# Hanbo-Cheng/DAWN-pytorch

Hardware: NVIDIA H100
Metric: denoising-steps/sec (200-frame 256^2 clip) (higher is better)
Workload: dtype f32

## Files before the change

dawn_pytorch_b200/_lib.py:

```python
import ctypes
import os

_HERE = os.path.dirname(os.path.abspath(__file__))
LIB_PATH = os.path.join(_HERE, "libdawn_unet.so")


class DawnUnetCfg(ctypes.Structure):
    _fields_ = [("dim", ctypes.c_int), ("n_levels", ctypes.c_int), ("dim_mults", ctypes.c_int * 8),
                ("channels", ctypes.c_int), ("cond_aud", ctypes.c_int), ("cond_pose", ctypes.c_int),
                ("cond_eye", ctypes.c_int), ("out_grid_dim", ctypes.c_int), ("out_conf_dim", ctypes.c_int),
                ("attn_heads", ctypes.c_int), ("attn_dim_head", ctypes.c_int), ("resnet_groups", ctypes.c_int),
                ("init_kernel_size", ctypes.c_int), ("win_width", ctypes.c_int)]


class DawnLfgCfg(ctypes.Structure):
    _fields_ = [("num_channels", ctypes.c_int), ("block_expansion", ctypes.c_int), ("max_features", ctypes.c_int),
                ("num_down_blocks", ctypes.c_int), ("num_bottleneck_blocks", ctypes.c_int), ("skips", ctypes.c_int)]


PATH_MMA_SYNC, PATH_TC_GEMM, PATH_TC_GEMM_PRESPLIT, PATH_TC_CONV3, PATH_TC_CONV3_TMA = range(5)
EPI_PLAIN, EPI_QKV_TEMPORAL, EPI_QKV_SLA, EPI_QKV_MID, EPI_CA_GATE, EPI_GN_APPLY = range(6)


class DawnContractionCase(ctypes.Structure):
    _i, _p = ctypes.c_int, ctypes.c_void_p
    _fields_ = [("path", _i), ("epi", _i),
                ("F", _i), ("IH", _i), ("IW", _i), ("Cin", _i), ("lda", _i),
                ("ntaps", _i), ("dy", _i * 52), ("dx", _i * 52), ("in_stride", _i),
                ("OHs", _i), ("OWs", _i), ("OH", _i), ("OW", _i), ("out_stride", _i), ("oy0", _i), ("ox0", _i),
                ("up2", _i),
                ("perm_pb", _i), ("perm_F", _i), ("perm_in", _i), ("perm_out", _i), ("perm_f_lo", _i), ("perm_f_hi", _i),
                ("P", _i),
                ("N", _i), ("ldb", _i), ("ldo", _i), ("ldr", _i), ("drain", _i), ("ln_inline", _i),
                ("rows_per_batch", _i), ("b_batch_stride", ctypes.c_longlong), ("cpg", _i),
                ("q_post_scale", ctypes.c_float),
                ("A", _p), ("B", _p), ("bias", _p), ("Res", _p), ("Out", _p),
                ("stats", _p), ("rowstats", _p), ("wsum", _p), ("rot", _p),
                ("kq", _p), ("nkq", _p), ("gates", _p),
                ("Y", _p), ("ldy", _i), ("gn_stats", _p), ("gn_w", _p), ("gn_b", _p), ("film", _p), ("gn_count", ctypes.c_double)]


FUSED_TEMPORAL, FUSED_ATTN_TC, FUSED_ATTN_SIMT, FUSED_SLA_CTX, FUSED_SLA_OUT, FUSED_SLA_CTX_UNFUSED, FUSED_CA_WT, \
    FUSED_CA_RSTD, FUSED_GN_HCOND, FUSED_TEMPORAL_MMA_SYNC = range(10)


class DawnFusedCase(ctypes.Structure):
    _i, _p = ctypes.c_int, ctypes.c_void_p
    _fields_ = [("kernel", _i), ("F", _i), ("P", _i), ("C", _i), ("band", _i), ("q_lo", _i), ("q_hi", _i),
                ("nseq", _i), ("L", _i), ("pb", _i), ("seq_base_stride", ctypes.c_longlong), ("elem_stride", ctypes.c_longlong),
                ("ldx", _i), ("ldr", _i), ("ldo", _i), ("ld", _i), ("ldb", _i), ("ldy", _i), ("ldbT", _i),
                ("x", _p), ("res", _p), ("out", _p), ("gamma", _p), ("w_qkv", _p), ("w_out", _p), ("rot", _p), ("bias", _p),
                ("qkv", _p), ("Bf", _p), ("out_bias", _p), ("kq", _p), ("nkq", _p), ("G", _p), ("gates", _p), ("Wt", _p),
                ("T", _p), ("Y", _p), ("out16h", _p), ("out16l", _p),
                ("gn_stats", _p), ("gn_count", ctypes.c_double), ("cpg", _i), ("gn_w", _p), ("gn_b", _p), ("film", _p)]
# ... 182 lines not shown
```

dawn_pytorch_b200/csrc/contraction.cu:

```cuda
#include <algorithm>
#include <cstring>

#include "common.cuh"
#include "contraction.cuh"
#include "kernels.cuh"
#include "tc_gemm.cuh"

namespace dawn {

void HostParams::set(const std::string& name, const float* data, const int64_t* shape, int ndim) {
  HostParam p;
  p.shape.assign(shape, shape + ndim);
  int64_t numel = 1;
  for (int64_t s : p.shape) numel *= s;
  p.data.assign(data, data + numel);
  map[name] = std::move(p);
}

int HostParams::need(const std::string& name, const std::vector<int64_t>& shape, const HostParam** out) const {
  auto it = map.find(name);
  if (it == map.end()) { set_last_error(prefix + "missing parameter: " + name); return -1; }
  const HostParam& p = it->second;
  if (p.shape != shape) {
    std::string s = prefix + "parameter " + name + " has shape (";
// ... 217 lines not shown

  GemmParams p;
  memset(&p, 0, sizeof(p));
  p.A = c.A; p.lda = c.lda; p.Cin = c.Cin;
  p.up2 = c.up2;
  p.IH = c.IH; p.IW = c.IW; p.OHs = c.OHs; p.OWs = c.OWs; p.in_stride = c.in_stride;
  p.ntaps = c.ntaps;
  for (int t = 0; t < c.ntaps; ++t) { p.dy[t] = (signed char)c.dy[t]; p.dx[t] = (signed char)c.dx[t]; }
  p.M = c.F * c.OHs * c.OWs; p.N = c.N; p.K = c.ntaps * c.Cin;
  p.rows_per_batch = c.rows_per_batch > 0 ? c.rows_per_batch : p.M;
  p.perm_pb = c.perm_pb; p.perm_F = c.perm_F; p.perm_in = c.perm_in; p.perm_out = c.perm_out;
  p.perm_f_lo = c.perm_f_lo; p.perm_f_hi = c.perm_f_hi;
  p.B = c.B; p.ldb = c.ldb; p.b_batch_stride = c.b_batch_stride;
  p.Out = c.Out; p.ldo = c.ldo; p.OH = c.OH; p.OW = c.OW; p.out_stride = c.out_stride; p.oy0 = c.oy0; p.ox0 = c.ox0;
  p.bias = c.bias; p.Res = c.Res; p.ldr = c.ldr;
  p.stats = c.stats; p.cpg = c.cpg; p.clips = 1;
  p.rowstats = c.rowstats; p.ln_inline = c.ln_inline; p.wsum = c.wsum; p.rot = c.rot; p.P = c.P;
  p.q_post_scale = c.q_post_scale;
  p.kq = c.kq; p.nkq = c.nkq; p.gates = c.gates;
  p.Y = c.Y; p.ldy = c.ldy; p.gn_stats = c.gn_stats; p.gn_w = c.gn_w; p.gn_b = c.gn_b; p.film = c.film; p.gn_count = c.gn_count;
  p.drain = c.drain;

  const bool ln = c.epi >= EPI_QKV_TEMPORAL && c.epi <= EPI_CA_GATE;
  if (p.ln_inline && (c.path != DAWN_PATH_TC_GEMM || p.ntaps != 1)) return refuse("inline LayerNorm statistics need the gather-producer wgmma GEMM and one tap");
  if (ln && !p.ln_inline && !p.rowstats) return refuse("LayerNorm epilogue without row statistics");
  if (ln && !p.wsum) return refuse("LayerNorm epilogue without wsum");
  if (c.epi == EPI_PLAIN && p.stats && (p.cpg <= 0 || p.N / p.cpg > 8)) return refuse("GroupNorm statistics need 8 groups");

  Owned own;
  if (c.path != DAWN_PATH_MMA_SYNC) {
    std::vector<float> hB((size_t)p.K * p.ldb);
    DAWN_CUDA_OK(cudaMemcpy(hB.data(), p.B, hB.size() * sizeof(float), cudaMemcpyDeviceToHost));
    PackedWeight w;
    DAWN_TRY(upload_weight(own.v, hB, p.K, p.N, p.ldb, {}, &w));
    set_weights(p, w);
    p.bias = c.bias;
  }
  const bool split = c.path == DAWN_PATH_TC_GEMM_PRESPLIT || c.path == DAWN_PATH_TC_CONV3_TMA;
  const size_t scratch_bytes = split ? (size_t)split_rows(p) * p.Cin * 4 : 0;
  if (!path_ok(p, c.epi, c.path, scratch_bytes)) return refuse("the path does not accept this geometry");
  float* scratch = nullptr;
  if (split) DAWN_TRY(dev_alloc(own.v, scratch_bytes / sizeof(float), &scratch));
// ... 13 lines not shown
```

dawn_pytorch_b200/csrc/tc_common.cuh:

```cuda
#pragma once
#include <type_traits>
#include "common.cuh"

namespace dawn {
namespace tc {

__device__ __forceinline__ uint32_t smem_u32(const void* p) { return (uint32_t)__cvta_generic_to_shared(p); }

__device__ __forceinline__ uint8_t* smem_align1024(uint8_t* base) { return base + ((1024u - (smem_u32(base) & 1023u)) & 1023u); }

template <uint32_t R>
__device__ __forceinline__ void setmaxnreg_dec() { asm volatile("setmaxnreg.dec.sync.aligned.u32 %0;" ::"n"(R)); }
template <uint32_t R>
__device__ __forceinline__ void setmaxnreg_inc() { asm volatile("setmaxnreg.inc.sync.aligned.u32 %0;" ::"n"(R)); }

template <int I, int N, class F>
__device__ __forceinline__ void static_for(F&& f) {
  if constexpr (I < N) {
    f(std::integral_constant<int, I>{});
    static_for<I + 1, N>(f);
  }
}

__device__ __forceinline__ void mbar_init(uint64_t* bar, uint32_t count) {
// ... 59 lines not shown
      "setp.ne.b32 p, %50, 0;\n\t"
      "wgmma.mma_async.sync.aligned.m64n96k16.f32.f16.f16 "
      "{%0, %1, %2, %3, %4, %5, %6, %7, %8, %9, %10, %11, %12, %13, %14, %15, "
      "%16, %17, %18, %19, %20, %21, %22, %23, %24, %25, %26, %27, %28, %29, %30, %31, "
      "%32, %33, %34, %35, %36, %37, %38, %39, %40, %41, %42, %43, %44, %45, %46, %47}, %48, %49, p, 1, 1, 0, 0;\n\t"
      "}"
      : "+f"(d[0]), "+f"(d[1]), "+f"(d[2]), "+f"(d[3]), "+f"(d[4]), "+f"(d[5]), "+f"(d[6]), "+f"(d[7]), "+f"(d[8]), "+f"(d[9]),
        "+f"(d[10]), "+f"(d[11]), "+f"(d[12]), "+f"(d[13]), "+f"(d[14]), "+f"(d[15]), "+f"(d[16]), "+f"(d[17]), "+f"(d[18]),
        "+f"(d[19]), "+f"(d[20]), "+f"(d[21]), "+f"(d[22]), "+f"(d[23]), "+f"(d[24]), "+f"(d[25]), "+f"(d[26]), "+f"(d[27]),
        "+f"(d[28]), "+f"(d[29]), "+f"(d[30]), "+f"(d[31]), "+f"(d[32]), "+f"(d[33]), "+f"(d[34]), "+f"(d[35]), "+f"(d[36]),
        "+f"(d[37]), "+f"(d[38]), "+f"(d[39]), "+f"(d[40]), "+f"(d[41]), "+f"(d[42]), "+f"(d[43]), "+f"(d[44]), "+f"(d[45]),
        "+f"(d[46]), "+f"(d[47])
      : "l"(adesc), "l"(bdesc), "r"(scale_d)
      : "memory");
}
__device__ __forceinline__ void wgmma_m64n64k16_rs(float (&d)[32], const uint32_t (&a)[4], uint64_t bdesc, uint32_t scale_d) {
  asm volatile(
      "{\n\t"
      ".reg .pred p;\n\t"
      "setp.ne.b32 p, %37, 0;\n\t"
      "wgmma.mma_async.sync.aligned.m64n64k16.f32.f16.f16 "
      "{%0, %1, %2, %3, %4, %5, %6, %7, %8, %9, %10, %11, %12, %13, %14, %15, "
      "%16, %17, %18, %19, %20, %21, %22, %23, %24, %25, %26, %27, %28, %29, %30, %31}, {%32, %33, %34, %35}, %36, p, 1, 1, 0;\n\t"
      "}"
      : "+f"(d[0]), "+f"(d[1]), "+f"(d[2]), "+f"(d[3]), "+f"(d[4]), "+f"(d[5]), "+f"(d[6]), "+f"(d[7]), "+f"(d[8]), "+f"(d[9]),
        "+f"(d[10]), "+f"(d[11]), "+f"(d[12]), "+f"(d[13]), "+f"(d[14]), "+f"(d[15]), "+f"(d[16]), "+f"(d[17]), "+f"(d[18]),
        "+f"(d[19]), "+f"(d[20]), "+f"(d[21]), "+f"(d[22]), "+f"(d[23]), "+f"(d[24]), "+f"(d[25]), "+f"(d[26]), "+f"(d[27]),
        "+f"(d[28]), "+f"(d[29]), "+f"(d[30]), "+f"(d[31])
      : "r"(a[0]), "r"(a[1]), "r"(a[2]), "r"(a[3]), "l"(bdesc), "r"(scale_d)
      : "memory");
}

__device__ __forceinline__ uint64_t make_desc(uint32_t saddr, uint32_t sbo = 1024) {
  return (uint64_t)((saddr >> 4) & 0x3FFF) | (1ull << 16) | ((uint64_t)((sbo >> 4) & 0x3FFF) << 32) | (1ull << 62);
}

constexpr int kStageLd = 68;
__device__ __forceinline__ void stage_fragment(float* stage, int r0, const float (&d)[32], bool first, int wtid) {
  const int w = wtid >> 5, l = wtid & 31;
  float* p0 = stage + (size_t)(r0 + w * 16 + (l >> 2)) * kStageLd + 2 * (l & 3);
  float* p1 = p0 + 8 * kStageLd;
#pragma unroll
  for (int j = 0; j < 8; ++j) {
    float2* a = reinterpret_cast<float2*>(p0 + 8 * j);
    float2* b = reinterpret_cast<float2*>(p1 + 8 * j);
    if (first) {
      *a = make_float2(d[4 * j], d[4 * j + 1]);
      *b = make_float2(d[4 * j + 2], d[4 * j + 3]);
    } else {
      const float2 x = *a, y = *b;
      *a = make_float2(x.x + d[4 * j], x.y + d[4 * j + 1]);
      *b = make_float2(y.x + d[4 * j + 2], y.y + d[4 * j + 3]);
    }
  }
}

__device__ __forceinline__ uint32_t swz(int r, int c) { return (uint32_t)((r >> 3) * 1024 + (r & 7) * 128 + ((c ^ (r & 7)) << 4)); }

__device__ __forceinline__ void store_rows_coalesced(float* wbuf, const float (&acc)[64], float* out, size_t opix, int ldo,
                                                     int n0, bool rv, int lane) {
  float* dst[4];
#pragma unroll
  for (int k = 0; k < 4; ++k) {
    const int r = (lane >> 2) + 8 * k;
    const uint32_t lo = __shfl_sync(0xffffffffu, (uint32_t)opix, r);
    const uint32_t hi = __shfl_sync(0xffffffffu, (uint32_t)((unsigned long long)opix >> 32), r);
    const int ok = __shfl_sync(0xffffffffu, rv ? 1 : 0, r);
// ... 23 lines not shown
```

dawn_pytorch_b200/csrc/tc_conv3.cu:

```cuda
#include <cuda.h>
#include <cuda_fp16.h>
#include <cstdlib>
#include <cstring>
#include <string>
#include <map>
#include <tuple>
#include "common.cuh"
#include "f16x3.cuh"
#include "gemm.cuh"
#include "tc_common.cuh"
#include "tc_gemm.cuh"

namespace dawn {
namespace {

using namespace tc;

constexpr int TH = 16, TW = 8;
constexpr int HH = TH + 2, HW = TW + 2;
constexpr int NPROD = 256;
constexpr int PAIR_HH = 8 + 2;
constexpr int PAIR_ROW_B = 104;

template <int BN, bool PAIR = false>
struct CCfg {
  static_assert(!PAIR || BN == 64, "the pair-mode halos fit next to 64-column weight stages only");
  static constexpr int NWG = BN / 64;
  static constexpr bool SPLIT_EPI = (BN == 64);
  static constexpr int B_PANEL = BN * 128;
  static constexpr int FRAME_ROWS = PAIR ? PAIR_HH * HW : HH * HW;
  static constexpr int HALO_ROWS = PAIR ? PAIR_ROW_B + FRAME_ROWS : FRAME_ROWS;
  static constexpr int A_HALO = (HALO_ROWS * 128 + 1023) / 1024 * 1024;
  static constexpr int A_STAGES = 2;
  static constexpr int B_STAGES = PAIR ? 3 : (BN == 64) ? 4 : 2;
  static constexpr int A_BYTES = A_STAGES * 2 * A_HALO;
  static constexpr int B_BYTES = B_STAGES * 2 * B_PANEL;
  static constexpr int ACC_STAGE = 2 * 128 * kStageLd * 4;
  static constexpr int SMEM_DYN = A_BYTES + B_BYTES + ACC_STAGE + 1024;
  static_assert(SMEM_DYN + 1024 <= 232448, "shared memory");
  static constexpr int EPI_WARP = NPROD / 32 + 4 * NWG;
  static constexpr int LOAD_WARP = EPI_WARP + (SPLIT_EPI ? 4 : 0);
  static constexpr int NTHREADS = 32 * LOAD_WARP + 128;
  static constexpr uint32_t REG_LAUNCH = (65536 / NTHREADS) & ~7u;
  static constexpr uint32_t REG_LOAD = 24, REG_MMA = SPLIT_EPI ? 136 : 128, REG_EPI = 128;
  static_assert(REG_LOAD < REG_LAUNCH && REG_MMA > REG_LAUNCH && REG_EPI > REG_LAUNCH, "register budgets");
  static_assert(2 * REG_LAUNCH + REG_LOAD + NWG * REG_MMA + (SPLIT_EPI ? REG_EPI : 0) <= NTHREADS / 128 * REG_LAUNCH, "CTA register pool");
};

template <int BN, bool TMA, bool PAIR>
__device__ __forceinline__ void tc_conv3_body(const GemmParams& p, const float* __restrict__ Bimg, int tiles_y, int tiles_x, int tiles_n,
                                              int img_bn, const CUtensorMap& tm_hi, const CUtensorMap& tm_lo) {
  using C = CCfg<BN, PAIR>;
  constexpr int B_PANEL = C::B_PANEL, A_STAGES = C::A_STAGES, B_STAGES = C::B_STAGES, NWG = C::NWG;
  constexpr int A_HALO = C::A_HALO, FRAME_ROWS = C::FRAME_ROWS;
  constexpr bool SPLIT = C::SPLIT_EPI;
  extern __shared__ uint8_t smem_raw[];
  __shared__ uint64_t a_full[A_STAGES], a_free[A_STAGES], b_full[B_STAGES], b_free[B_STAGES];
  __shared__ uint64_t st_full[2], st_free[2];
  __shared__ float s_stat[NWG][16];
  __shared__ __align__(16) float s_bias[NWG][64];

  const int tid = threadIdx.x, lane = tid & 31;
  const int warp = __shfl_sync(0xffffffffu, tid >> 5, 0);
  uint8_t* smem = smem_align1024(smem_raw);
  uint8_t* smemA = smem;
  uint8_t* smemB = smem + C::A_BYTES;
  float* stage_base = reinterpret_cast<float*>(smemB + C::B_BYTES);

  if (tid == 0) {
    for (int s = 0; s < A_STAGES; ++s) { mbar_init(&a_full[s], TMA ? 1 : NPROD); mbar_init(&a_free[s], 4 * NWG); }
    for (int s = 0; s < B_STAGES; ++s) { mbar_init(&b_full[s], 1); mbar_init(&b_free[s], 4 * NWG); }
    for (int s = 0; s < 2; ++s) { mbar_init(&st_full[s], 128); mbar_init(&st_free[s], 128); }
    asm volatile("fence.mbarrier_init.release.cluster;" ::: "memory");
  }
  __syncthreads();
// ... 134 lines not shown
            if (PAIR) {
              bulk_copy_g2s(smemB + s * 2 * B_PANEL, panel, B_PANEL, &b_full[s]);
              bulk_copy_g2s(smemB + s * 2 * B_PANEL + B_PANEL, panel + ipanel, B_PANEL, &b_full[s]);
            } else {
              bulk_copy_g2s(smemB + s * 2 * B_PANEL, panel, 2 * B_PANEL, &b_full[s]);
            }
          }
      }
    }
    return;
  }

  const int wg = SPLIT ? 0 : (warp - 8) >> 2;
  const int ew = (warp - 8) & 3;
  const int etid = ew * 32 + lane;
  const int bar_id = 2 + wg;
  constexpr uint32_t SBO_HALO = HW * 128;
  constexpr uint32_t H2 = PAIR ? PAIR_ROW_B * 128 : 8 * HW * 128;
  const int dt = (p.drain == 1 || p.drain == 3) ? p.drain : 9;

  auto mma_tile = [&](auto DTc, float* stage, uint32_t& ait, uint32_t& bit, auto&& claim) {
    constexpr int DT = decltype(DTc)::value;
    float d0[32], d1[32];
    bool first_drain = true;
    for (int cc = 0; cc < NCH; ++cc, ++ait) {
      const int sa = ait % A_STAGES;
      mbar_wait(&a_full[sa], (ait / A_STAGES) & 1);
      fence_proxy_async();
      const uint32_t a_hi = smem_u32(smemA + sa * 2 * A_HALO), a_lo = a_hi + A_HALO;
      static_for<0, 9>([&](auto TAPc) {
        constexpr int tap = decltype(TAPc)::value;
        constexpr bool group_first = tap % DT == 0, group_last = tap % DT == DT - 1;
        constexpr uint32_t woff = (uint32_t)(((tap / 3) * HW + tap % 3) * 128);
        const int sb = bit % B_STAGES;
        const int sprev = (bit + B_STAGES - 1) % B_STAGES;
        mbar_wait(&b_full[sb], (bit / B_STAGES) & 1);
        const uint64_t ahi = make_desc(a_hi + woff, SBO_HALO), alo = make_desc(a_lo + woff, SBO_HALO);
        const uint64_t ahi2 = make_desc(a_hi + woff + H2, SBO_HALO), alo2 = make_desc(a_lo + woff + H2, SBO_HALO);
        const uint32_t sbaddr = smem_u32(smemB + sb * 2 * B_PANEL) + wg * 64 * 128;
        const uint64_t bhi = make_desc(sbaddr), blo = make_desc(sbaddr + B_PANEL);
        wgmma_fence();
#pragma unroll
        for (int j = 0; j < 4; ++j) {
          const uint64_t o = (uint64_t)(j * 2);
          const uint32_t acc = (group_first && j == 0) ? 0u : 1u;
          wgmma_m64n64k16(d0, alo + o, bhi + o, acc);
          wgmma_m64n64k16(d1, alo2 + o, bhi + o, acc);
          wgmma_m64n64k16(d0, ahi + o, blo + o, 1u);
          wgmma_m64n64k16(d1, ahi2 + o, blo + o, 1u);
          wgmma_m64n64k16(d0, ahi + o, bhi + o, 1u);
          wgmma_m64n64k16(d1, ahi2 + o, bhi + o, 1u);
        }
        wgmma_commit();
        if constexpr (group_last) {
          wgmma_wait<0>();
          wgmma_fence_acc(d0); wgmma_fence_acc(d1);
          if (lane == 0) { if (!group_first) mbar_arrive(&b_free[sprev]); mbar_arrive(&b_free[sb]); }
          if (first_drain) claim();
          stage_fragment(stage, 0, d0, first_drain, etid);
          stage_fragment(stage, 64, d1, first_drain, etid);
          first_drain = false;
        } else {
          wgmma_wait<1>();
          wgmma_fence_acc(d0); wgmma_fence_acc(d1);
          if (lane == 0 && !group_first) mbar_arrive(&b_free[sprev]);
        }
        ++bit;
      });
      if (lane == 0) mbar_arrive(&a_free[sa]);
    }
  };

  const bool defer_stats = (p.stats != nullptr) && tiles_n == 1;
  const bool bias_smem = (p.bias != nullptr) && tiles_n == 1;
  auto load_bias = [&]() {
    if (bias_smem) {
      if (etid < 64) s_bias[wg][etid] = __ldg(p.bias + wg * 64 + etid);
      asm volatile("bar.sync %0, 128;" ::"r"(bar_id) : "memory");
    }
  };
  auto flush_stats = [&](float (&gs)[8], float (&gss)[8], int clip) {
    const int n0f = wg * 64;
    double* cs = p.stats + 16 * clip;
#pragma unroll
    for (int b8 = 0; b8 < 8; ++b8) {
      double s = (double)gs[b8], ss = (double)gss[b8];
#pragma unroll
      for (int o = 16; o > 0; o >>= 1) { s += __shfl_xor_sync(0xffffffffu, s, o); ss += __shfl_xor_sync(0xffffffffu, ss, o); }
      if (lane == 0) {
        const int grp = (n0f + b8 * 8) / p.cpg;
        atomicAdd(&cs[2 * grp], s);
        atomicAdd(&cs[2 * grp + 1], ss);
      }
      gs[b8] = 0.f; gss[b8] = 0.f;
    }
  };
  auto epilogue_tile = [&](int tile, float* stage, float (&gs)[8], float (&gss)[8], int& pending, int& pclip) {
    int f, y0, x0, nt, nf;
    decode(tile, f, y0, x0, nt, nf);
    const int clip = p.clips > 1 ? f % p.clips : 0;
    const int n0 = nt * BN + wg * 64;
    const int row_in_tile = etid;
    float* s_st = s_stat[wg];
    float* wbuf = stage + ew * 32 * kStageLd;
    float acc[64];
    {
      const float4* src = reinterpret_cast<const float4*>(stage + row_in_tile * kStageLd);
#pragma unroll
      for (int i = 0; i < 16; ++i) {
        const float4 v = src[i];
        acc[4 * i] = v.x; acc[4 * i + 1] = v.y; acc[4 * i + 2] = v.z; acc[4 * i + 3] = v.w;
      }
    }
    __syncwarp();
#pragma unroll
    for (int i = 0; i < 64; ++i) acc[i] *= p.tc_scale;
    const int fr = PAIR ? row_in_tile >> 6 : 0;
    const int img = f + fr * p.clips;
    const int oy = y0 + ((row_in_tile >> 3) & (PAIR ? 7 : 15)), ox = x0 + (row_in_tile & 7);
    const bool rv = (oy < H) && (ox < W) && fr < nf;
    size_t opix = (size_t)img * H * W + (size_t)(rv ? oy * W + ox : 0);
    int ocol = n0;
    if (p.up2) {
      const int cls = n0 >> 6, py = cls >> 1, px = cls & 1;
      opix = (size_t)img * 4 * H * W + (size_t)(rv ? (2 * oy + py) * 2 * W + 2 * ox + px : 0);
      ocol = n0 & 63;
    }
    if (bias_smem) {
      const float4* bp = reinterpret_cast<const float4*>(s_bias[wg]);
#pragma unroll
      for (int i = 0; i < 16; ++i) {
        const float4 b = bp[i];
        acc[4 * i] += b.x; acc[4 * i + 1] += b.y; acc[4 * i + 2] += b.z; acc[4 * i + 3] += b.w;
      }
    } else if (p.bias) {
      const float4* bp = reinterpret_cast<const float4*>(p.bias + n0);
#pragma unroll
      for (int i = 0; i < 16; ++i) {
        const float4 b = __ldg(bp + i);
        acc[4 * i] += b.x; acc[4 * i + 1] += b.y; acc[4 * i + 2] += b.z; acc[4 * i + 3] += b.w;
      }
    }
    store_rows_coalesced(wbuf, acc, p.Out, opix, p.ldo, ocol, rv, lane);
    if (defer_stats) {
// ... 17 lines not shown
        float s = 0.f, ss = 0.f;
        if (rv) {
#pragma unroll
          for (int i = 0; i < 8; ++i) { const float x = acc[b8 * 8 + i]; s += x; ss += x * x; }
        }
        s = warp_sum(s); ss = warp_sum(ss);
        if (lane == 0) {
          const int grp = (n0 + b8 * 8) / p.cpg;
          atomicAdd(&s_st[2 * grp], s);
          atomicAdd(&s_st[2 * grp + 1], ss);
        }
      }
      asm volatile("bar.sync %0, 128;" ::"r"(bar_id) : "memory");
      if (etid < 16) {
        const int grp = etid >> 1;
        const int glo = n0 / p.cpg, ghi = (n0 + 63) / p.cpg;
        if (grp >= glo && grp <= ghi) atomicAdd(&p.stats[16 * clip + etid], (double)s_st[etid]);
      }
    }
  };
  auto with_drain = [&](auto&& run) {
    if (dt == 1) run(std::integral_constant<int, 1>{});
    else if (dt == 3) run(std::integral_constant<int, 3>{});
    else run(std::integral_constant<int, 9>{});
  };

  if (SPLIT && warp >= C::EPI_WARP) {
    setmaxnreg_inc<C::REG_EPI>();
    float gs[8], gss[8];
    int pending = 0, pclip = 0;
#pragma unroll
// ... 12 lines not shown
    with_drain([&](auto DTc) {
      uint32_t ait = 0, bit = 0, lt = 0;
      for (int tile = blockIdx.x; tile < total_tiles; tile += gridDim.x, ++lt) {
        const int b = lt & 1;
        mma_tile(DTc, stage_base + b * 128 * kStageLd, ait, bit, [&]() { mbar_wait(&st_free[b], ((lt >> 1) & 1) ^ 1); });
        mbar_arrive(&st_full[b]);
      }
    });
  } else {
    setmaxnreg_inc<C::REG_MMA>();
    float gs[8], gss[8];
    int pending = 0, pclip = 0;
#pragma unroll
    for (int i = 0; i < 8; ++i) { gs[i] = 0.f; gss[i] = 0.f; }
    load_bias();
    float* stage = stage_base + wg * 128 * kStageLd;
    uint32_t ait = 0, bit = 0;
    for (int tile = blockIdx.x; tile < total_tiles; tile += gridDim.x) {
      with_drain([&](auto DTc) { mma_tile(DTc, stage, ait, bit, []() {}); });
      asm volatile("bar.sync %0, 128;" ::"r"(bar_id) : "memory");
      epilogue_tile(tile, stage, gs, gss, pending, pclip);
      asm volatile("bar.sync %0, 128;" ::"r"(bar_id) : "memory");
    }
    if (defer_stats && pending > 0) flush_stats(gs, gss, pclip);
  }
}

template <int BN, bool TMA>
__global__ void __launch_bounds__(CCfg<BN>::NTHREADS, 1) tc_conv3_kernel(const GemmParams p, const float* __restrict__ Bimg,
                                                                          int tiles_y, int tiles_x, int tiles_n, int img_bn,
                                                                          const __grid_constant__ CUtensorMap tm_hi,
                                                                          const __grid_constant__ CUtensorMap tm_lo) {
  tc_conv3_body<BN, TMA, false>(p, Bimg, tiles_y, tiles_x, tiles_n, img_bn, tm_hi, tm_lo);
}

template <bool TMA>
// ... 103 lines not shown
```

dawn_pytorch_b200/csrc/tc_gemm.cu:

```cuda
#include <cuda_fp16.h>
#include "common.cuh"
#include "f16x3.cuh"
#include "gemm.cuh"
#include "tc_common.cuh"
#include "tc_gemm.cuh"

namespace dawn {
namespace {

constexpr int BM = 128;
constexpr int BKP = 64;
constexpr int CHUNK = 4;
constexpr int A_PANEL_MIN = BM * 128;
constexpr int NPROD = 256;

template <int BN>
struct Cfg {
  static constexpr int NWG = BN / 64;
  static constexpr int A_PANEL = A_PANEL_MIN;
  static constexpr int B_PANEL = BN * 128;
  static constexpr int STAGE_BYTES = 2 * A_PANEL + 2 * B_PANEL;
  static constexpr int STAGES = (BN == 64) ? 3 : 2;
  static constexpr int LOAD_WARP = (NPROD + 128 * NWG) / 32;
  static constexpr int NTHREADS = 32 * LOAD_WARP + 128;
// ... 199 lines not shown
        const int nt = tile % tiles_n;
        const uint8_t* src = reinterpret_cast<const uint8_t*>(Bimg) + (size_t)nt * KC * (2 * B_PANEL);
        for (int kc = 0; kc < KC; ++kc, ++it) {
          const int s = it % STAGES;
          const uint32_t round = it / STAGES;
          mbar_wait(&slot_free[s], (round & 1) ^ 1);
          mbar_arrive_expect_tx(&b_full[s], 2 * B_PANEL);
          bulk_copy_g2s(smem + s * STAGE_BYTES + 2 * A_PANEL, src + (size_t)kc * (2 * B_PANEL), 2 * B_PANEL, &b_full[s]);
        }
      }
    }
  } else {
    setmaxnreg_inc<C::REG_MMA>();
    const int wg = (warp - 8) >> 2;
    const int ew = (warp - 8) & 3;
    const int row_in_tile = ew * 32 + lane;
    const int etid = (tid - NPROD) & 127;
    float* s_st = s_stat[wg];
    const int bar_id = 2 + wg;
    constexpr int EN = 64;
    float* stage = reinterpret_cast<float*>(smem + STAGES * STAGE_BYTES) + wg * BM * kStageLd;
    float* wbuf = stage + ew * 32 * kStageLd;
    int Te = -1;
    const bool bias_s = (p.bias != nullptr) && p.N <= 1024;
    if (bias_s) {
      for (int i = (tid - NPROD); i < p.N; i += 128 * NWG) s_biasv[i] = __ldg(p.bias + i);
      asm volatile("bar.sync 4, %0;" ::"n"(128 * NWG) : "memory");
    }
    const int CH = (p.drain > 0 && p.drain < CHUNK) ? p.drain : CHUNK;
    auto mma_chunk = [&](auto NPc, float* stage, uint32_t& it, bool first) {
      constexpr int NP = decltype(NPc)::value;
      float d0[32], d1[32];
      static_for<0, NP>([&](auto Ic) {
        constexpr int i = decltype(Ic)::value;
        const int s = it % STAGES;
        const int sprev = (it + STAGES - 1) % STAGES;
        const uint32_t round = it / STAGES;
        mbar_wait(&a_full[s], round & 1);
        mbar_wait(&b_full[s], round & 1);
        fence_proxy_async();
        const uint32_t sa = smem_u32(smem + s * STAGE_BYTES);
        const uint64_t ahi = make_desc(sa), alo = make_desc(sa + A_PANEL);
        const uint64_t bhi = make_desc(sa + 2 * A_PANEL + wg * 64 * 128), blo = make_desc(sa + 2 * A_PANEL + B_PANEL + wg * 64 * 128);
        constexpr uint64_t H2 = 64 * 128 / 16;
        wgmma_fence();
#pragma unroll
        for (int j = 0; j < BKP / 16; ++j) {
          const uint64_t o = (uint64_t)(j * 2);
          const uint32_t acc = (i == 0 && j == 0) ? 0u : 1u;
          wgmma_m64n64k16(d0, alo + o, bhi + o, acc);
          wgmma_m64n64k16(d1, alo + H2 + o, bhi + o, acc);
          wgmma_m64n64k16(d0, ahi + o, blo + o, 1u);
          wgmma_m64n64k16(d1, ahi + H2 + o, blo + o, 1u);
          wgmma_m64n64k16(d0, ahi + o, bhi + o, 1u);
          wgmma_m64n64k16(d1, ahi + H2 + o, bhi + o, 1u);
        }
        wgmma_commit();
        if constexpr (i == NP - 1) {
          wgmma_wait<0>();
          wgmma_fence_acc(d0); wgmma_fence_acc(d1);
          if (lane == 0) { if (i > 0) mbar_arrive(&slot_free[sprev]); mbar_arrive(&slot_free[s]); }
          stage_fragment(stage, 0, d0, first, etid);
          stage_fragment(stage, 64, d1, first, etid);
        } else {
          wgmma_wait<1>();
          wgmma_fence_acc(d0); wgmma_fence_acc(d1);
          if (lane == 0 && i > 0) mbar_arrive(&slot_free[sprev]);
        }
        ++it;
      });
    };
    static_assert(CHUNK == 4, "the chunk dispatch below expands 1 .. 4 panels");
    uint32_t it = 0;
    for (int tile = blockIdx.x; tile < total_tiles; tile += gridDim.x) {
      ++Te;
      const int m0 = (tile / tiles_n) * BM, n0 = (tile % tiles_n) * BN + wg * EN;
      for (int kc = 0; kc < KC; kc += CH) {
        const int np = min(CH, KC - kc);
        if (np == 4) mma_chunk(std::integral_constant<int, 4>{}, stage, it, kc == 0);
        else if (np == 3) mma_chunk(std::integral_constant<int, 3>{}, stage, it, kc == 0);
        else if (np == 2) mma_chunk(std::integral_constant<int, 2>{}, stage, it, kc == 0);
        else mma_chunk(std::integral_constant<int, 1>{}, stage, it, kc == 0);
      }
      asm volatile("bar.sync %0, 128;" ::"r"(bar_id) : "memory");
      float acc[EN];
      {
        const float4* src = reinterpret_cast<const float4*>(stage + row_in_tile * kStageLd);
#pragma unroll
        for (int i = 0; i < EN / 4; ++i) {
          const float4 v = src[i];
          acc[4 * i] = v.x; acc[4 * i + 1] = v.y; acc[4 * i + 2] = v.z; acc[4 * i + 3] = v.w;
        }
      }
      __syncwarp();

      const int m = m0 + row_in_tile;
      bool rv = m < p.M;
      const int mc = rv ? m : (p.M - 1);
      int opx = 0;
      if (p.perm_out) {
        opx = seq_blocked_out_pixel(mc, p.perm_pb, p.perm_F, p.P, p.perm_f_lo, p.perm_f_hi);
        if (opx < 0) { rv = false; opx = 0; }
// ... 67 lines not shown
            float s = 0.f, ss = 0.f;
            if (rv) {
#pragma unroll
              for (int i = 0; i < 8; ++i) { const float x = acc[b8 * 8 + i]; s += x; ss += x * x; }
            }
            s = warp_sum(s); ss = warp_sum(ss);
            if (lane == 0) {
              const int grp = (n0 + b8 * 8) / p.cpg;
              atomicAdd(&s_st[2 * grp], s);
              atomicAdd(&s_st[2 * grp + 1], ss);
            }
          }
          asm volatile("bar.sync %0, 128;" ::"r"(bar_id) : "memory");
          if (etid < 16) {
            const int grp = etid >> 1;
            const int glo = n0 / p.cpg, ghi = (n0 + EN - 1) / p.cpg;
            if (grp >= glo && grp <= ghi) atomicAdd(&cs[etid], (double)s_st[etid]);
          }
        }
      } else {
        float mu, rs;
        if (p.ln_inline) { const float2 st = s_ln[Te & 7][row_in_tile]; mu = st.x; rs = st.y; }
        else { mu = p.rowstats[2 * (size_t)srow]; rs = p.rowstats[2 * (size_t)srow + 1]; }
        {
          const float fa = rs * p.tc_scale, fb = -rs * mu;
          const float4* wp = reinterpret_cast<const float4*>(p.wsum + n0);
#pragma unroll
          for (int i = 0; i < EN / 4; ++i) {
            const float4 w = __ldg(wp + i);
            acc[4 * i] = fmaf(fb, w.x, fa * acc[4 * i]); acc[4 * i + 1] = fmaf(fb, w.y, fa * acc[4 * i + 1]);
            acc[4 * i + 2] = fmaf(fb, w.z, fa * acc[4 * i + 2]); acc[4 * i + 3] = fmaf(fb, w.w, fa * acc[4 * i + 3]);
// ... 139 lines not shown
```

include/dawn_unet.h:

```cpp
#ifndef DAWN_UNET_H_
#define DAWN_UNET_H_

#include <stdint.h>

#ifdef __cplusplus
extern "C" {
#endif

typedef struct dawn_unet dawn_unet;

typedef struct {
  int dim;
  int n_levels;
  int dim_mults[8];
  int channels;
  int cond_aud;
  int cond_pose;
  int cond_eye;
  int out_grid_dim;
  int out_conf_dim;
  int attn_heads;
  int attn_dim_head;
  int resnet_groups;
  int init_kernel_size;
// ... 74 lines not shown
  int up2;
  int perm_pb, perm_F, perm_in, perm_out, perm_f_lo, perm_f_hi;
  int P;
  int N, ldb, ldo, ldr, drain, ln_inline;
  int rows_per_batch;
  long long b_batch_stride;
  int cpg;
  float q_post_scale;
  const float* A; const float* B; const float* bias; const float* Res; float* Out;
  double* stats;
  const float* rowstats;
  const float* wsum;
  const float* rot;
  const float* kq; const float* nkq; float* gates;
  const float* Y; int ldy; const double* gn_stats; const float* gn_w; const float* gn_b; const float* film; double gn_count;
} dawn_contraction_case;
int dawn_test_contraction(const dawn_contraction_case* c, void* stream);

enum {
  DAWN_FUSED_TEMPORAL = 0,
  DAWN_FUSED_ATTN_TC = 1,
  DAWN_FUSED_ATTN_SIMT = 2,
  DAWN_FUSED_SLA_CTX = 3,
  DAWN_FUSED_SLA_OUT = 4,
  DAWN_FUSED_SLA_CTX_UNFUSED = 5,
  DAWN_FUSED_CA_WT = 6,
  DAWN_FUSED_CA_RSTD = 7,
  DAWN_FUSED_GN_HCOND = 8,
  DAWN_FUSED_TEMPORAL_MMA_SYNC = 9
};
// ... 71 lines not shown
```

Baseline: 22.45.

## Split two-warpgroup wgmma tiles by rows with m64n128 instructions instead of columns

When two consumer warpgroups share a tile, each now takes one 64-row half of the M tile and issues m64n128k16 wgmma over the full 128-wide N tile, rather than each taking 64 columns with pairs of m64n64 instructions. This halves the number of wgmma issues per K step and changes how B descriptors are shared. The staging, epilogue row and column mapping, bias loads and GroupNorm group ranges are remapped to match. A clips field is added to the test contraction interface to exercise interleaved clips. Each thread now holds a 64-float accumulator array, which may raise register pressure.

```diff
diff --git a/dawn_pytorch_b200/_lib.py b/dawn_pytorch_b200/_lib.py
--- a/dawn_pytorch_b200/_lib.py
+++ b/dawn_pytorch_b200/_lib.py
@@ -37,7 +37,8 @@
                 ("A", _p), ("B", _p), ("bias", _p), ("Res", _p), ("Out", _p),
                 ("stats", _p), ("rowstats", _p), ("wsum", _p), ("rot", _p),
                 ("kq", _p), ("nkq", _p), ("gates", _p),
-                ("Y", _p), ("ldy", _i), ("gn_stats", _p), ("gn_w", _p), ("gn_b", _p), ("film", _p), ("gn_count", ctypes.c_double)]
+                ("Y", _p), ("ldy", _i), ("gn_stats", _p), ("gn_w", _p), ("gn_b", _p), ("film", _p), ("gn_count", ctypes.c_double),
+                ("clips", _i)]
 
 
 FUSED_TEMPORAL, FUSED_ATTN_TC, FUSED_ATTN_SIMT, FUSED_SLA_CTX, FUSED_SLA_OUT, FUSED_SLA_CTX_UNFUSED, FUSED_CA_WT, \
diff --git a/dawn_pytorch_b200/csrc/contraction.cu b/dawn_pytorch_b200/csrc/contraction.cu
--- a/dawn_pytorch_b200/csrc/contraction.cu
+++ b/dawn_pytorch_b200/csrc/contraction.cu
@@ -255,7 +255,7 @@
   p.B = c.B; p.ldb = c.ldb; p.b_batch_stride = c.b_batch_stride;
   p.Out = c.Out; p.ldo = c.ldo; p.OH = c.OH; p.OW = c.OW; p.out_stride = c.out_stride; p.oy0 = c.oy0; p.ox0 = c.ox0;
   p.bias = c.bias; p.Res = c.Res; p.ldr = c.ldr;
-  p.stats = c.stats; p.cpg = c.cpg; p.clips = 1;
+  p.stats = c.stats; p.cpg = c.cpg; p.clips = c.clips > 1 ? c.clips : 1;
   p.rowstats = c.rowstats; p.ln_inline = c.ln_inline; p.wsum = c.wsum; p.rot = c.rot; p.P = c.P;
   p.q_post_scale = c.q_post_scale;
   p.kq = c.kq; p.nkq = c.nkq; p.gates = c.gates;
@@ -267,6 +267,8 @@
   if (ln && !p.ln_inline && !p.rowstats) return refuse("LayerNorm epilogue without row statistics");
   if (ln && !p.wsum) return refuse("LayerNorm epilogue without wsum");
   if (c.epi == EPI_PLAIN && p.stats && (p.cpg <= 0 || p.N / p.cpg > 8)) return refuse("GroupNorm statistics need 8 groups");
+  if (p.clips > 1 && (c.F % p.clips != 0 || c.epi != EPI_PLAIN || c.perm_in || c.perm_out || c.path == DAWN_PATH_MMA_SYNC))
+    return refuse("interleaved clips need whole clips of frames and the plain epilogue of a wgmma path");
 
   Owned own;
   if (c.path != DAWN_PATH_MMA_SYNC) {
diff --git a/dawn_pytorch_b200/csrc/tc_common.cuh b/dawn_pytorch_b200/csrc/tc_common.cuh
--- a/dawn_pytorch_b200/csrc/tc_common.cuh
+++ b/dawn_pytorch_b200/csrc/tc_common.cuh
@@ -97,6 +97,27 @@
       : "l"(adesc), "l"(bdesc), "r"(scale_d)
       : "memory");
 }
+__device__ __forceinline__ void wgmma_m64n128k16(float (&d)[64], uint64_t adesc, uint64_t bdesc, uint32_t scale_d) {
+  asm volatile(
+      "{\n\t"
+      ".reg .pred p;\n\t"
+      "setp.ne.b32 p, %66, 0;\n\t"
+      "wgmma.mma_async.sync.aligned.m64n128k16.f32.f16.f16 "
+      "{%0, %1, %2, %3, %4, %5, %6, %7, %8, %9, %10, %11, %12, %13, %14, %15, "
+      "%16, %17, %18, %19, %20, %21, %22, %23, %24, %25, %26, %27, %28, %29, %30, %31, "
+      "%32, %33, %34, %35, %36, %37, %38, %39, %40, %41, %42, %43, %44, %45, %46, %47, "
+      "%48, %49, %50, %51, %52, %53, %54, %55, %56, %57, %58, %59, %60, %61, %62, %63}, %64, %65, p, 1, 1, 0, 0;\n\t"
+      "}"
+      : "+f"(d[0]), "+f"(d[1]), "+f"(d[2]), "+f"(d[3]), "+f"(d[4]), "+f"(d[5]), "+f"(d[6]), "+f"(d[7]), "+f"(d[8]), "+f"(d[9]),
+        "+f"(d[10]), "+f"(d[11]), "+f"(d[12]), "+f"(d[13]), "+f"(d[14]), "+f"(d[15]), "+f"(d[16]), "+f"(d[17]), "+f"(d[18]),
+        "+f"(d[19]), "+f"(d[20]), "+f"(d[21]), "+f"(d[22]), "+f"(d[23]), "+f"(d[24]), "+f"(d[25]), "+f"(d[26]), "+f"(d[27]),
+        "+f"(d[28]), "+f"(d[29]), "+f"(d[30]), "+f"(d[31]), "+f"(d[32]), "+f"(d[33]), "+f"(d[34]), "+f"(d[35]), "+f"(d[36]),
+        "+f"(d[37]), "+f"(d[38]), "+f"(d[39]), "+f"(d[40]), "+f"(d[41]), "+f"(d[42]), "+f"(d[43]), "+f"(d[44]), "+f"(d[45]),
+        "+f"(d[46]), "+f"(d[47]), "+f"(d[48]), "+f"(d[49]), "+f"(d[50]), "+f"(d[51]), "+f"(d[52]), "+f"(d[53]), "+f"(d[54]),
+        "+f"(d[55]), "+f"(d[56]), "+f"(d[57]), "+f"(d[58]), "+f"(d[59]), "+f"(d[60]), "+f"(d[61]), "+f"(d[62]), "+f"(d[63])
+      : "l"(adesc), "l"(bdesc), "r"(scale_d)
+      : "memory");
+}
 __device__ __forceinline__ void wgmma_m64n64k16_rs(float (&d)[32], const uint32_t (&a)[4], uint64_t bdesc, uint32_t scale_d) {
   asm volatile(
       "{\n\t"
@@ -119,21 +140,24 @@
 }
 
 constexpr int kStageLd = 68;
-__device__ __forceinline__ void stage_fragment(float* stage, int r0, const float (&d)[32], bool first, int wtid) {
+template <int H = 0, int N>
+__device__ __forceinline__ void stage_fragment(float* stage, int r0, const float (&d)[N], bool first, int wtid) {
+  static_assert(32 * (H + 1) <= N, "column half outside the fragment");
   const int w = wtid >> 5, l = wtid & 31;
   float* p0 = stage + (size_t)(r0 + w * 16 + (l >> 2)) * kStageLd + 2 * (l & 3);
   float* p1 = p0 + 8 * kStageLd;
 #pragma unroll
   for (int j = 0; j < 8; ++j) {
+    const int i = 32 * H + 4 * j;
     float2* a = reinterpret_cast<float2*>(p0 + 8 * j);
     float2* b = reinterpret_cast<float2*>(p1 + 8 * j);
     if (first) {
-      *a = make_float2(d[4 * j], d[4 * j + 1]);
-      *b = make_float2(d[4 * j + 2], d[4 * j + 3]);
+      *a = make_float2(d[i], d[i + 1]);
+      *b = make_float2(d[i + 2], d[i + 3]);
     } else {
       const float2 x = *a, y = *b;
-      *a = make_float2(x.x + d[4 * j], x.y + d[4 * j + 1]);
-      *b = make_float2(y.x + d[4 * j + 2], y.y + d[4 * j + 3]);
+      *a = make_float2(x.x + d[i], x.y + d[i + 1]);
+      *b = make_float2(y.x + d[i + 2], y.y + d[i + 3]);
     }
   }
 }
diff --git a/dawn_pytorch_b200/csrc/tc_conv3.cu b/dawn_pytorch_b200/csrc/tc_conv3.cu
--- a/dawn_pytorch_b200/csrc/tc_conv3.cu
+++ b/dawn_pytorch_b200/csrc/tc_conv3.cu
@@ -37,7 +37,7 @@
   static constexpr int B_BYTES = B_STAGES * 2 * B_PANEL;
   static constexpr int ACC_STAGE = 2 * 128 * kStageLd * 4;
   static constexpr int SMEM_DYN = A_BYTES + B_BYTES + ACC_STAGE + 1024;
-  static_assert(SMEM_DYN + 1024 <= 232448, "shared memory");
+  static_assert(SMEM_DYN + 2048 <= 232448, "shared memory");
   static constexpr int EPI_WARP = NPROD / 32 + 4 * NWG;
   static constexpr int LOAD_WARP = EPI_WARP + (SPLIT_EPI ? 4 : 0);
   static constexpr int NTHREADS = 32 * LOAD_WARP + 128;
@@ -58,7 +58,7 @@
   __shared__ uint64_t a_full[A_STAGES], a_free[A_STAGES], b_full[B_STAGES], b_free[B_STAGES];
   __shared__ uint64_t st_full[2], st_free[2];
   __shared__ float s_stat[NWG][16];
-  __shared__ __align__(16) float s_bias[NWG][64];
+  __shared__ __align__(16) float s_bias[NWG][BN];
 
   const int tid = threadIdx.x, lane = tid & 31;
   const int warp = __shfl_sync(0xffffffffu, tid >> 5, 0);
@@ -223,6 +223,8 @@
   const int wg = SPLIT ? 0 : (warp - 8) >> 2;
   const int ew = (warp - 8) & 3;
   const int etid = ew * 32 + lane;
+  const int ch = NWG == 2 ? ew >> 1 : 0;
+  const int erow = NWG == 2 ? 64 * wg + (etid & 63) : etid;
   const int bar_id = 2 + wg;
   constexpr uint32_t SBO_HALO = HW * 128;
   constexpr uint32_t H2 = PAIR ? PAIR_ROW_B * 128 : 8 * HW * 128;
@@ -231,6 +233,11 @@
   auto mma_tile = [&](auto DTc, float* stage, uint32_t& ait, uint32_t& bit, auto&& claim) {
     constexpr int DT = decltype(DTc)::value;
     float d0[32], d1[32];
+    float d[64];
+    auto fence_acc = [&]() {
+      if constexpr (NWG == 2) wgmma_fence_acc(d);
+      else { wgmma_fence_acc(d0); wgmma_fence_acc(d1); }
+    };
     bool first_drain = true;
     for (int cc = 0; cc < NCH; ++cc, ++ait) {
       const int sa = ait % A_STAGES;
@@ -244,34 +251,52 @@
         const int sb = bit % B_STAGES;
         const int sprev = (bit + B_STAGES - 1) % B_STAGES;
         mbar_wait(&b_full[sb], (bit / B_STAGES) & 1);
-        const uint64_t ahi = make_desc(a_hi + woff, SBO_HALO), alo = make_desc(a_lo + woff, SBO_HALO);
-        const uint64_t ahi2 = make_desc(a_hi + woff + H2, SBO_HALO), alo2 = make_desc(a_lo + woff + H2, SBO_HALO);
-        const uint32_t sbaddr = smem_u32(smemB + sb * 2 * B_PANEL) + wg * 64 * 128;
+        const uint32_t sbaddr = smem_u32(smemB + sb * 2 * B_PANEL);
         const uint64_t bhi = make_desc(sbaddr), blo = make_desc(sbaddr + B_PANEL);
         wgmma_fence();
-#pragma unroll
-        for (int j = 0; j < 4; ++j) {
-          const uint64_t o = (uint64_t)(j * 2);
-          const uint32_t acc = (group_first && j == 0) ? 0u : 1u;
-          wgmma_m64n64k16(d0, alo + o, bhi + o, acc);
-          wgmma_m64n64k16(d1, alo2 + o, bhi + o, acc);
-          wgmma_m64n64k16(d0, ahi + o, blo + o, 1u);
-          wgmma_m64n64k16(d1, ahi2 + o, blo + o, 1u);
-          wgmma_m64n64k16(d0, ahi + o, bhi + o, 1u);
-          wgmma_m64n64k16(d1, ahi2 + o, bhi + o, 1u);
+        if constexpr (NWG == 2) {
+          const uint32_t aw = woff + wg * H2;
+          const uint64_t ahi = make_desc(a_hi + aw, SBO_HALO), alo = make_desc(a_lo + aw, SBO_HALO);
+#pragma unroll
+          for (int j = 0; j < 4; ++j) {
+            const uint64_t o = (uint64_t)(j * 2);
+            const uint32_t acc = (group_first && j == 0) ? 0u : 1u;
+            wgmma_m64n128k16(d, alo + o, bhi + o, acc);
+            wgmma_m64n128k16(d, ahi + o, blo + o, 1u);
+            wgmma_m64n128k16(d, ahi + o, bhi + o, 1u);
+          }
+        } else {
+          const uint64_t ahi = make_desc(a_hi + woff, SBO_HALO), alo = make_desc(a_lo + woff, SBO_HALO);
+          const uint64_t ahi2 = make_desc(a_hi + woff + H2, SBO_HALO), alo2 = make_desc(a_lo + woff + H2, SBO_HALO);
+#pragma unroll
+          for (int j = 0; j < 4; ++j) {
+            const uint64_t o = (uint64_t)(j * 2);
+            const uint32_t acc = (group_first && j == 0) ? 0u : 1u;
+            wgmma_m64n64k16(d0, alo + o, bhi + o, acc);
+            wgmma_m64n64k16(d1, alo2 + o, bhi + o, acc);
+            wgmma_m64n64k16(d0, ahi + o, blo + o, 1u);
+            wgmma_m64n64k16(d1, ahi2 + o, blo + o, 1u);
+            wgmma_m64n64k16(d0, ahi + o, bhi + o, 1u);
+            wgmma_m64n64k16(d1, ahi2 + o, bhi + o, 1u);
+          }
         }
         wgmma_commit();
         if constexpr (group_last) {
           wgmma_wait<0>();
-          wgmma_fence_acc(d0); wgmma_fence_acc(d1);
+          fence_acc();
           if (lane == 0) { if (!group_first) mbar_arrive(&b_free[sprev]); mbar_arrive(&b_free[sb]); }
           if (first_drain) claim();
-          stage_fragment(stage, 0, d0, first_drain, etid);
-          stage_fragment(stage, 64, d1, first_drain, etid);
+          if constexpr (NWG == 2) {
+            stage_fragment<0>(stage, 64 * wg, d, first_drain, etid);
+            stage_fragment<1>(stage + 128 * kStageLd, 64 * wg, d, first_drain, etid);
+          } else {
+            stage_fragment(stage, 0, d0, first_drain, etid);
+            stage_fragment(stage, 64, d1, first_drain, etid);
+          }
           first_drain = false;
         } else {
           wgmma_wait<1>();
-          wgmma_fence_acc(d0); wgmma_fence_acc(d1);
+          fence_acc();
           if (lane == 0 && !group_first) mbar_arrive(&b_free[sprev]);
         }
         ++bit;
@@ -284,12 +309,12 @@
   const bool bias_smem = (p.bias != nullptr) && tiles_n == 1;
   auto load_bias = [&]() {
     if (bias_smem) {
-      if (etid < 64) s_bias[wg][etid] = __ldg(p.bias + wg * 64 + etid);
+      if (etid < BN) s_bias[wg][etid] = __ldg(p.bias + etid);
       asm volatile("bar.sync %0, 128;" ::"r"(bar_id) : "memory");
     }
   };
   auto flush_stats = [&](float (&gs)[8], float (&gss)[8], int clip) {
-    const int n0f = wg * 64;
+    const int n0f = ch * 64;
     double* cs = p.stats + 16 * clip;
 #pragma unroll
     for (int b8 = 0; b8 < 8; ++b8) {
@@ -308,10 +333,11 @@
     int f, y0, x0, nt, nf;
     decode(tile, f, y0, x0, nt, nf);
     const int clip = p.clips > 1 ? f % p.clips : 0;
-    const int n0 = nt * BN + wg * 64;
-    const int row_in_tile = etid;
+    const int n0 = nt * BN + ch * 64;
+    const int row_in_tile = erow;
     float* s_st = s_stat[wg];
-    float* wbuf = stage + ew * 32 * kStageLd;
+    stage += ch * 128 * kStageLd;
+    float* wbuf = stage + (row_in_tile - lane) * kStageLd;
     float acc[64];
     {
       const float4* src = reinterpret_cast<const float4*>(stage + row_in_tile * kStageLd);
@@ -336,7 +362,7 @@
       ocol = n0 & 63;
     }
     if (bias_smem) {
-      const float4* bp = reinterpret_cast<const float4*>(s_bias[wg]);
+      const float4* bp = reinterpret_cast<const float4*>(s_bias[wg] + ch * 64);
 #pragma unroll
       for (int i = 0; i < 16; ++i) {
         const float4 b = bp[i];
@@ -384,7 +410,7 @@
       asm volatile("bar.sync %0, 128;" ::"r"(bar_id) : "memory");
       if (etid < 16) {
         const int grp = etid >> 1;
-        const int glo = n0 / p.cpg, ghi = (n0 + 63) / p.cpg;
+        const int glo = nt * BN / p.cpg, ghi = (nt * BN + BN - 1) / p.cpg;
         if (grp >= glo && grp <= ghi) atomicAdd(&p.stats[16 * clip + etid], (double)s_st[etid]);
       }
     }
@@ -427,12 +453,11 @@
 #pragma unroll
     for (int i = 0; i < 8; ++i) { gs[i] = 0.f; gss[i] = 0.f; }
     load_bias();
-    float* stage = stage_base + wg * 128 * kStageLd;
     uint32_t ait = 0, bit = 0;
     for (int tile = blockIdx.x; tile < total_tiles; tile += gridDim.x) {
-      with_drain([&](auto DTc) { mma_tile(DTc, stage, ait, bit, []() {}); });
+      with_drain([&](auto DTc) { mma_tile(DTc, stage_base, ait, bit, []() {}); });
       asm volatile("bar.sync %0, 128;" ::"r"(bar_id) : "memory");
-      epilogue_tile(tile, stage, gs, gss, pending, pclip);
+      epilogue_tile(tile, stage_base, gs, gss, pending, pclip);
       asm volatile("bar.sync %0, 128;" ::"r"(bar_id) : "memory");
     }
     if (defer_stats && pending > 0) flush_stats(gs, gss, pclip);
diff --git a/dawn_pytorch_b200/csrc/tc_gemm.cu b/dawn_pytorch_b200/csrc/tc_gemm.cu
--- a/dawn_pytorch_b200/csrc/tc_gemm.cu
+++ b/dawn_pytorch_b200/csrc/tc_gemm.cu
@@ -237,13 +237,15 @@
     setmaxnreg_inc<C::REG_MMA>();
     const int wg = (warp - 8) >> 2;
     const int ew = (warp - 8) & 3;
-    const int row_in_tile = ew * 32 + lane;
+    const int ch = NWG == 2 ? ew >> 1 : 0;
+    const int row_in_tile = NWG == 2 ? 64 * wg + 32 * (ew & 1) + lane : ew * 32 + lane;
     const int etid = (tid - NPROD) & 127;
     float* s_st = s_stat[wg];
     const int bar_id = 2 + wg;
     constexpr int EN = 64;
-    float* stage = reinterpret_cast<float*>(smem + STAGES * STAGE_BYTES) + wg * BM * kStageLd;
-    float* wbuf = stage + ew * 32 * kStageLd;
+    float* stage = reinterpret_cast<float*>(smem + STAGES * STAGE_BYTES);
+    float* estage = stage + ch * BM * kStageLd;
+    float* wbuf = estage + (row_in_tile - lane) * kStageLd;
     int Te = -1;
     const bool bias_s = (p.bias != nullptr) && p.N <= 1024;
     if (bias_s) {
@@ -254,6 +256,11 @@
     auto mma_chunk = [&](auto NPc, float* stage, uint32_t& it, bool first) {
       constexpr int NP = decltype(NPc)::value;
       float d0[32], d1[32];
+      float d[64];
+      auto fence_acc = [&]() {
+        if constexpr (NWG == 2) wgmma_fence_acc(d);
+        else { wgmma_fence_acc(d0); wgmma_fence_acc(d1); }
+      };
       static_for<0, NP>([&](auto Ic) {
         constexpr int i = decltype(Ic)::value;
         const int s = it % STAGES;
@@ -263,31 +270,49 @@
         mbar_wait(&b_full[s], round & 1);
         fence_proxy_async();
         const uint32_t sa = smem_u32(smem + s * STAGE_BYTES);
-        const uint64_t ahi = make_desc(sa), alo = make_desc(sa + A_PANEL);
-        const uint64_t bhi = make_desc(sa + 2 * A_PANEL + wg * 64 * 128), blo = make_desc(sa + 2 * A_PANEL + B_PANEL + wg * 64 * 128);
         constexpr uint64_t H2 = 64 * 128 / 16;
         wgmma_fence();
-#pragma unroll
-        for (int j = 0; j < BKP / 16; ++j) {
-          const uint64_t o = (uint64_t)(j * 2);
-          const uint32_t acc = (i == 0 && j == 0) ? 0u : 1u;
-          wgmma_m64n64k16(d0, alo + o, bhi + o, acc);
-          wgmma_m64n64k16(d1, alo + H2 + o, bhi + o, acc);
-          wgmma_m64n64k16(d0, ahi + o, blo + o, 1u);
-          wgmma_m64n64k16(d1, ahi + H2 + o, blo + o, 1u);
-          wgmma_m64n64k16(d0, ahi + o, bhi + o, 1u);
-          wgmma_m64n64k16(d1, ahi + H2 + o, bhi + o, 1u);
+        if constexpr (NWG == 2) {
+          const uint64_t ahi = make_desc(sa) + wg * H2, alo = make_desc(sa + A_PANEL) + wg * H2;
+          const uint64_t bhi = make_desc(sa + 2 * A_PANEL), blo = make_desc(sa + 2 * A_PANEL + B_PANEL);
+#pragma unroll
+          for (int j = 0; j < BKP / 16; ++j) {
+            const uint64_t o = (uint64_t)(j * 2);
+            const uint32_t acc = (i == 0 && j == 0) ? 0u : 1u;
+            wgmma_m64n128k16(d, alo + o, bhi + o, acc);
+            wgmma_m64n128k16(d, ahi + o, blo + o, 1u);
+            wgmma_m64n128k16(d, ahi + o, bhi + o, 1u);
+          }
+        } else {
+          const uint64_t ahi = make_desc(sa), alo = make_desc(sa + A_PANEL);
+          const uint64_t bhi = make_desc(sa + 2 * A_PANEL), blo = make_desc(sa + 2 * A_PANEL + B_PANEL);
+#pragma unroll
+          for (int j = 0; j < BKP / 16; ++j) {
+            const uint64_t o = (uint64_t)(j * 2);
+            const uint32_t acc = (i == 0 && j == 0) ? 0u : 1u;
+            wgmma_m64n64k16(d0, alo + o, bhi + o, acc);
+            wgmma_m64n64k16(d1, alo + H2 + o, bhi + o, acc);
+            wgmma_m64n64k16(d0, ahi + o, blo + o, 1u);
+            wgmma_m64n64k16(d1, ahi + H2 + o, blo + o, 1u);
+            wgmma_m64n64k16(d0, ahi + o, bhi + o, 1u);
+            wgmma_m64n64k16(d1, ahi + H2 + o, bhi + o, 1u);
+          }
         }
         wgmma_commit();
         if constexpr (i == NP - 1) {
           wgmma_wait<0>();
-          wgmma_fence_acc(d0); wgmma_fence_acc(d1);
+          fence_acc();
           if (lane == 0) { if (i > 0) mbar_arrive(&slot_free[sprev]); mbar_arrive(&slot_free[s]); }
-          stage_fragment(stage, 0, d0, first, etid);
-          stage_fragment(stage, 64, d1, first, etid);
+          if constexpr (NWG == 2) {
+            stage_fragment<0>(stage, 64 * wg, d, first, etid);
+            stage_fragment<1>(stage + BM * kStageLd, 64 * wg, d, first, etid);
+          } else {
+            stage_fragment(stage, 0, d0, first, etid);
+            stage_fragment(stage, 64, d1, first, etid);
+          }
         } else {
           wgmma_wait<1>();
-          wgmma_fence_acc(d0); wgmma_fence_acc(d1);
+          fence_acc();
           if (lane == 0 && i > 0) mbar_arrive(&slot_free[sprev]);
         }
         ++it;
@@ -297,7 +322,7 @@
     uint32_t it = 0;
     for (int tile = blockIdx.x; tile < total_tiles; tile += gridDim.x) {
       ++Te;
-      const int m0 = (tile / tiles_n) * BM, n0 = (tile % tiles_n) * BN + wg * EN;
+      const int m0 = (tile / tiles_n) * BM, n0 = (tile % tiles_n) * BN + ch * EN;
       for (int kc = 0; kc < KC; kc += CH) {
         const int np = min(CH, KC - kc);
         if (np == 4) mma_chunk(std::integral_constant<int, 4>{}, stage, it, kc == 0);
@@ -308,7 +333,7 @@
       asm volatile("bar.sync %0, 128;" ::"r"(bar_id) : "memory");
       float acc[EN];
       {
-        const float4* src = reinterpret_cast<const float4*>(stage + row_in_tile * kStageLd);
+        const float4* src = reinterpret_cast<const float4*>(estage + row_in_tile * kStageLd);
 #pragma unroll
         for (int i = 0; i < EN / 4; ++i) {
           const float4 v = src[i];
@@ -406,7 +431,8 @@
           asm volatile("bar.sync %0, 128;" ::"r"(bar_id) : "memory");
           if (etid < 16) {
             const int grp = etid >> 1;
-            const int glo = n0 / p.cpg, ghi = (n0 + EN - 1) / p.cpg;
+            const int n0w = (tile % tiles_n) * BN;
+            const int glo = n0w / p.cpg, ghi = (n0w + BN - 1) / p.cpg;
             if (grp >= glo && grp <= ghi) atomicAdd(&cs[etid], (double)s_st[etid]);
           }
         }
diff --git a/include/dawn_unet.h b/include/dawn_unet.h
--- a/include/dawn_unet.h
+++ b/include/dawn_unet.h
@@ -112,6 +112,7 @@
   const float* rot;
   const float* kq; const float* nkq; float* gates;
   const float* Y; int ldy; const double* gn_stats; const float* gn_w; const float* gn_b; const float* film; double gn_count;
+  int clips;
 } dawn_contraction_case;
 int dawn_test_contraction(const dawn_contraction_case* c, void* stream);
 
```

After: 22.66, median of 6. About the same (+0.9%).
